# CalciferZh/MinimalOptiX

Hardware: AMD Instinct MI355X
Metric: Mrays/s (primary+bounce+shadow rays traced per second, coffee.obj 1920x1080 256spp) (higher is better)
Workload: dtype f32

## Files before the change

minimaloptix_amd/csrc/api_context.h:

```cpp
#pragma once
#include <hip/hip_runtime.h>

#include <initializer_list>
#include <string>
#include <vector>

#include "../../include/moptix.h"
#include "lbvh.h"
#include "megakernel.h"
#include "refitkernel.h"
#include "pt_signtopo.h"

struct ncclComm;

namespace pt { namespace api {

template <class T> struct DevBuf {
  T* p = nullptr; size_t n = 0;
  hipError_t ensure(size_t count) {
    if (count <= n && p) return hipSuccess;
    if (p) { (void)hipFree(p); p = nullptr; n = 0; }
    hipError_t e = hipMalloc((void**)&p, sizeof(T) * (count ? count : 1));
    if (e == hipSuccess) n = count ? count : 1;
    return e;
// ... 250 lines not shown
void fill_view(moptix_context c, SceneView& v);
int scene_features(moptix_context c);
int fill_query_view(moptix_context c, SceneView& v);
moptix_aov_buffers aov_ptrs(moptix_context c);
void comm_release(moptix_context c);
int denoise_begin(moptix_context c, bool ownGuide, size_t& px);
void denoise_consts(moptix_context c, const moptix_denoise_params* p, DenoiseConsts& k);
inline float* denoise_out(moptix_context c) { return c->dn.bound ? c->dn.bound : c->dn.out.p; }

struct LaunchPlan {
  const TraceKernel* kernel;
  int variant;
  int features;
  int nItems, tilesX;
  int nBlocks;
  long long perPass;
  int slotsInUse, auxDepth, drainBelow, ovfDepth;
  int tileMajor, unitShift; long long historyUnits;
  size_t poolBytes, overflowInts, workInts;
};
struct RenderLaunch {
  LaunchPlan p; LaunchArgs a;
  long long perPass;
  bool counted, fast;
};
struct PassOverride {
  const int* order; int nWork;
  hipError_t (*reduce)(hipStream_t stream, const LaunchArgs& a, void* user); void* user;
};
int prepare_launch(moptix_context c, int32_t nSeeds, bool counted, bool byPixelSlots, RenderLaunch& r);
int launch_pass(moptix_context c, RenderLaunch& r, const int* dSeeds, int n, const PassOverride* over);

}}
```

minimaloptix_amd/csrc/api_render.hip:

```cpp
#include <rocprim/rocprim.hpp>

#include <algorithm>
#include <cstdio>
#include <cstdlib>
#include <cstring>

#include "api_context.h"
#include "pt_lanestack.h"

using namespace pt;
using namespace pt::api;

namespace {

constexpr int kProbeWidth = 128;
int choose_node_format(moptix_context c) {
  c->formatDecided = true;
  c->nodeFormatUsed = 128;
  for (auto& v : c->probeCounts) v = 0;
  if (c->bvh.nNodes <= 0 || !c->bvh.nodes64) return MOPTIX_OK;
  if (c->opt.nodeFormat != 0) { c->nodeFormatUsed = c->opt.nodeFormat; return MOPTIX_OK; }
  SceneView v; fill_view(c, v);
  v.nodes64 = c->bvh.nodes64;
  const int w = std::min(kProbeWidth, v.width), h = std::max(1, (int)((long long)v.height * w / std::max(1, v.width)));
// ... 85 lines not shown
  const long long localTiles = (nTiles + c->nRanks - 1) / c->nRanks;
  if (localTiles * 64 > 0x7fffffffLL) return fail(c, MOPTIX_ERR_LIMIT, "frame too large");
  p.nItems = (int)(localTiles * 64); p.tilesX = tilesX;
  if (p.nItems == 0) return MOPTIX_OK;
  const long long budget = (long long)c->opt.sampleBufMB << 20;
  p.perPass = budget / ((long long)p.nItems * 12);
  p.nBlocks = c->numCUs * c->opt.blocksPerCU;
  const long long counterSlack = (long long)c->numCUs * std::max(4, c->opt.blocksPerCU) * 1024 + 65536;
  if ((long long)p.nItems + counterSlack > 0x7fffffffLL) return fail(c, MOPTIX_ERR_LIMIT, "frame too large");
  p.perPass = std::min(p.perPass, (0x7fffffffLL - counterSlack) / p.nItems);
  p.perPass = std::max(1LL, std::min(p.perPass, (long long)nSeeds));

  const bool hasTris = scene.rootRef != kEmptyRef;
  const bool analyticQueue = c->opt.analyticQueue >= 0 ? c->opt.analyticQueue != 0 : (c->spheres.size() + c->quads.size() >= 64);
  const bool packetOk = hasTris && scene.nLights <= 3 && !scene.anyDisneyAnalytic;
  const double nSamples = (double)p.nItems * (double)nSeeds;
  const bool autoPacket = nSamples >= 1.0e6 && nSeeds >= 16;
  const bool variantExplicit = c->opt.kernelVariant >= 0;
  const int variant = variantExplicit ? c->opt.kernelVariant : 3;
  const bool usePacket = packetOk && (variant == 4 || (!variantExplicit && c->opt.autoPacket != 0 && autoPacket));
  const bool useQueue = !usePacket && (byPixelSlots || ((variant >= 3) && (hasTris || analyticQueue)));
  p.kernel = usePacket ? &kPacketKernel : !useQueue ? nullptr : hasTris ? &kQueueKernel : &kLeanQueueKernel;
  p.variant = usePacket ? 4 : useQueue ? 3 : 0;
  p.features = (usePacket && c->opt.specialize != 0) ? scene_features(c) : FEAT_ALL;
  if (p.kernel == &kLeanQueueKernel && c->opt.blocksPerCU == 3) p.nBlocks = c->numCUs * 4;
  p.slotsInUse = c->opt.slotsInUse >= 0 ? c->opt.slotsInUse : (usePacket && c->opt.auxDepth > 0 && nSamples < 1.0e8 && c->glassFaceShare <= 0.5 ? packetkernel_slots() * 7 / 8 : 0);
  p.auxDepth = usePacket ? c->opt.auxDepth : 0;
  if (usePacket) {
    bool glassMaterial = false;
    for (const DevMaterial& m : c->mats) if (m.kind == MAT_DISNEY && m.brdfType == BRDF_GLASS) glassMaterial = true;
    p.drainBelow = (glassMaterial && !scene.shadowNearest) ? 0 : c->opt.drainBelow;
  }
  if (p.kernel) {
    p.ovfDepth = hasTris ? std::max(0, c->bvh.stackBound - p.kernel->lds_stack_entries() + 1) : 0;
    p.overflowInts = p.ovfDepth > 0 ? p.kernel->overflow_ints(p.nBlocks, p.ovfDepth) : 0;
    p.poolBytes = p.kernel->cold_bytes(p.nBlocks);
  } else {
    p.overflowInts = lane_stack_overflow_entries((size_t)p.nBlocks * 256, c->bvh.stackBound, megakernel_lds_stack_entries());
  }
  p.workInts = 2 + drain_list_ints(p.nBlocks, p.drainBelow);
  p.tileMajor = byPixelSlots ? 3 : p.kernel ? c->opt.tileMajor : 0;
  p.unitShift = p.tileMajor == 3 ? 0 : 6;
  p.historyUnits = (localTiles * 64) >> p.unitShift;
  return MOPTIX_OK;
}

int report_tile_history(moptix_context c) {
  std::vector<unsigned int> cost((size_t)c->tiles.units);
  HIPCHK(c, hipMemcpy(cost.data(), c->tiles.keys.p, sizeof(unsigned int) * cost.size(), hipMemcpyDeviceToHost), "read tile cost");
  size_t hist[6] = { 0, 0, 0, 0, 0, 0 };
  for (size_t i = 0; i < cost.size(); i++) {
    const unsigned int v = cost[i];
    hist[v == 0 ? 0 : v < 16 ? 1 : v < 64 ? 2 : v < 256 ? 3 : 4]++;
    if (v >= 256 && i < cost.size() / 2) hist[5]++;
  }
  fprintf(stderr, "[moptix] depth history (%zu units): none %zu, depth 8-15 %zu, 16-63 %zu, 64-255 %zu, capped %zu (of which %zu in the first half)\n",
          cost.size(), hist[0], hist[1], hist[2], hist[3], hist[4], hist[5]);
  return MOPTIX_OK;
}

#ifdef PT_EVLOG
constexpr size_t kEvLogWords = 65536;
int evlog_begin(moptix_context c, DevBuf<unsigned long long>& evLog, LaunchArgs& a) {
// ... 33 lines not shown
  a.starveLanes = c->opt.starveLanes; a.swapLanes = c->opt.swapLanes;
  a.slotsInUse = p.slotsInUse; a.auxDepth = p.auxDepth; a.ovfDepth = p.ovfDepth;
  a.watchdogTicks = (unsigned long long)c->opt.watchdogMs * 100000ull;
  if (p.overflowInts > 0) {
    HIPCHK(c, c->dOverflow.ensure(p.overflowInts), "alloc stack overflow area");
    a.stackOverflow = c->dOverflow.p;
  }
  if (p.kernel) {
    HIPCHK(c, c->dPoolCold.ensure(p.poolBytes), "alloc path pool");
    a.poolCold = c->dPoolCold.p;
  }
  long long perPass = p.perPass;
  for (;;) {
    const hipError_t e = c->dSampleBuf.ensure((size_t)perPass * a.nItems * 3);
    if (e == hipSuccess) break;
    if (e != hipErrorOutOfMemory || perPass <= 1) return hipFail(c, e, "alloc per-sample buffer");
    (void)hipGetLastError();
    perPass = (perPass + 1) / 2;
  }
  r.perPass = perPass;
  a.sampleBuf = c->dSampleBuf.p;
  HIPCHK(c, c->dWork.ensure(p.workInts), "alloc work counter");
  {
    const int hdr[2 + kDrainEntries] = { 0, 0, 0, 0, 0, 0, p.nBlocks * p.drainBelow, p.drainBelow };
    HIPCHK(c, hipMemcpyAsync(c->dWork.p, hdr, sizeof(hdr), hipMemcpyHostToDevice, c->stream), "init work counter");
    HIPCHK(c, hipStreamSynchronize(c->stream), "sync");
  }
  a.workCounter = c->dWork.p;
  a.tileMajor = p.tileMajor; a.unitShift = p.unitShift;
  if (p.tileMajor) {
    HIPCHK(c, c->tiles.ensure(p.historyUnits, c->stream), "start depth history");
    a.tileOrder = c->tiles.order.p; a.tileCost = c->tiles.keys.p;
  }
  if (counted) {
    HIPCHK(c, c->dCounters.ensure(kCntTotal), "alloc counters");
    HIPCHK(c, hipMemsetAsync(c->dCounters.p, 0, sizeof(unsigned long long) * kCntTotal, c->stream), "zero counters");
    HIPCHK(c, hipMemsetAsync(c->dCounters.p + kCntFirstWaveIn, 0xff, sizeof(unsigned long long) * 2, c->stream), "init min counters");
    a.counters = c->dCounters.p;
  }
  return MOPTIX_OK;
}

static hipError_t sort_pairs_desc(void* tmp, size_t& tmpBytes, OrderList& l, size_t n, hipStream_t stream) {
  return rocprim::radix_sort_pairs_desc(tmp, tmpBytes, l.keys.p, l.keysSorted.p, l.iota.p, l.order.p, n, 0, 32, stream);
}

hipError_t OrderList::ensure(long long n, hipStream_t stream) {
  if (units == n) return hipSuccess;
  units = -1;
  std::vector<int> ids((size_t)n);
  for (size_t i = 0; i < ids.size(); i++) ids[i] = (int)i;
  hipError_t e = keys.ensure((size_t)n);
  if (e == hipSuccess) e = keysSorted.ensure((size_t)n);
  if (e == hipSuccess) e = order.ensure((size_t)n);
  if (e == hipSuccess) e = iota.upload(ids, stream);
  if (e == hipSuccess) e = hipMemsetAsync(keys.p, 0, sizeof(unsigned int) * (size_t)n, stream);
  size_t tmpBytes = 0;
  if (e == hipSuccess) e = sort_pairs_desc(nullptr, tmpBytes, *this, (size_t)n, stream);
  if (e == hipSuccess) e = sortTmp.ensure(tmpBytes);
  if (e == hipSuccess) e = hipStreamSynchronize(stream);
  if (e == hipSuccess) units = n;
  return e;
}

hipError_t OrderList::sort(hipStream_t stream) {
  size_t tmpBytes = sortTmp.n;
  return sort_pairs_desc(sortTmp.p, tmpBytes, *this, (size_t)units, stream);
}

int launch_pass(moptix_context c, RenderLaunch& r, const int* dSeeds, int n, const PassOverride* over) {
  LaunchArgs& a = r.a;
  const LaunchPlan& p = r.p;
  a.seeds = dSeeds; a.nSeeds = n; a.nWork = over ? over->nWork : n * a.nItems;
  HIPCHK(c, hipMemsetAsync(c->dWork.p, 0, (2 + kDrainCap) * sizeof(int), c->stream), "zero work counter");
  if (over) a.tileOrder = over->order;
  else if (a.tileMajor && a.tileCost) HIPCHK(c, c->tiles.sort(c->stream), "sort tiles");
  HIPCHK(c, hipEventRecord(c->ev0, c->stream), "event");
  if (p.kernel) HIPCHK(c, p.kernel->launch(c->stream, a, p.nBlocks, r.counted, r.fast, p.features), p.kernel->launchWhat);
  else HIPCHK(c, launch_megakernel(c->stream, a, p.nBlocks, r.counted), "launch megakernel");
  if (p.drainBelow > 0) HIPCHK(c, launch_drainkernel(c->stream, a, c->numCUs, r.counted, r.fast), "launch drain kernel");
  else if (p.kernel == &kPacketKernel) HIPCHK(c, launch_megakernel(c->stream, a, p.nBlocks, r.counted), "launch megakernel");
  HIPCHK(c, hipEventRecord(c->ev1, c->stream), "event");
  if (over) HIPCHK(c, over->reduce(c->stream, a, over->user), "launch adaptive reduction");
  else HIPCHK(c, launch_reduce_samples(c->stream, a), "launch sample reduction");
  HIPCHK(c, hipEventRecord(c->ev2, c->stream), "event");
  c->asyncPending = true;
  return MOPTIX_OK;
}

}}

namespace {

int do_render(moptix_context c, const int32_t* seeds, int32_t nSeeds, bool counted, bool blocking, moptix_stats* stats) {
  int rc = check_ready(c);
  if (rc != MOPTIX_OK) return rc;
  if (nSeeds < 0 || (nSeeds > 0 && !seeds)) return fail(c, MOPTIX_ERR_INVALID, "bad seeds");
// ... 26 lines not shown
}

}

extern "C" {

int moptix_launch(moptix_context c, int32_t randSeed) { return do_render(c, &randSeed, 1, false, true, nullptr); }
int moptix_render(moptix_context c, const int32_t* seeds, int32_t nSeeds) { return do_render(c, seeds, nSeeds, false, true, nullptr); }
int moptix_render_async(moptix_context c, const int32_t* seeds, int32_t nSeeds) { return do_render(c, seeds, nSeeds, false, false, nullptr); }
int moptix_render_counted(moptix_context c, const int32_t* seeds, int32_t nSeeds, moptix_stats* out) {
  if (out) memset(out, 0, sizeof(*out));
  return do_render(c, seeds, nSeeds, true, true, out);
}

int moptix_sync(moptix_context c) {
  if (!c) return MOPTIX_ERR_INVALID;
  HIPCHK(c, hipStreamSynchronize(c->stream), "stream synchronize");
  if (c->asyncPending) {
    float ms = 0.f, ms2 = 0.f;
    if (hipEventElapsedTime(&ms, c->ev0, c->ev1) == hipSuccess) { c->kernelMs += ms; c->nLaunches++; }
    if (hipEventElapsedTime(&ms2, c->ev1, c->ev2) == hipSuccess) c->reduceMs += ms2;
    c->asyncPending = false;
    int flags[2] = { 0, 0 };
    if (c->dWork.p) HIPCHK(c, hipMemcpy(flags, c->dWork.p, sizeof(flags), hipMemcpyDeviceToHost), "read watchdog flag");
    if (flags[1] != 0) return fail(c, MOPTIX_ERR_HIP, "render kernel hit its watchdog (option watchdog_ms); this pass was not added to accuBuffer");
  }
  return MOPTIX_OK;
}

}
```

minimaloptix_amd/csrc/lbvh.hip:

```cpp
#include <cstring>
#include <utility>
#include <vector>
#include <hip/hip_runtime.h>
#include <rocprim/rocprim.hpp>

#include "lbvh.h"
#include "pt_lbvh.h"

namespace pt {

namespace {

constexpr int kBlock = 256;
inline int grid_for(int n) { return (n + kBlock - 1) / kBlock; }

struct SceneBox { uint32_t cLo[3], cHi[3], sLo[3], sHi[3]; };

constexpr int kReplicas = 64;
__global__ void k_init_box(SceneBox* b) {
  b += blockIdx.x;
  if (threadIdx.x < 3) {
    b->cLo[threadIdx.x] = float_to_ordered(1e37f); b->cHi[threadIdx.x] = float_to_ordered(-1e37f);
    b->sLo[threadIdx.x] = float_to_ordered(1e37f); b->sHi[threadIdx.x] = float_to_ordered(-1e37f);
  }
// ... 52 lines not shown
  const v3 shi = mk3(ordered_to_float(box->sHi[0]), ordered_to_float(box->sHi[1]), ordered_to_float(box->sHi[2]));
  keys[f] = morton_key(c, clo, invExt, lbvh_bits_per_axis(n), lbvh_index_bits(n), f) | (tri_is_big(l, h, slo, shi) ? 0ull : kSmallKeyBit);
}

__global__ void k_leaves(int n, const uint64_t* __restrict__ keys, const float* __restrict__ facePos,
                         const float* __restrict__ faceNrm, const int* __restrict__ faceHasNrm, const int* __restrict__ faceMat,
                         const float* __restrict__ lo, const float* __restrict__ hi, const SceneBox* box,
                         Tri48* __restrict__ tris, TriShade* __restrict__ shade, float* __restrict__ leafLo, float* __restrict__ leafHi) {
  const int k = blockIdx.x * blockDim.x + threadIdx.x;
  if (k >= n) return;
  const int f = key_face(keys[k], lbvh_index_bits(n));
  const float* p = facePos + 9 * (size_t)f;
  const v3 p0 = mk3(p[0], p[1], p[2]), p1 = mk3(p[3], p[4], p[5]), p2 = mk3(p[6], p[7], p[8]);
  Tri48 t;
  t.p0 = p0; t.e0 = p1 - p0; t.e1 = p0 - p2; t.mat = faceMat[f] & ((1 << kFaceMatBits) - 1); t.prim = f; t.shadow = faceMat[f] >> kFaceMatBits;
  tris[k] = t;
  TriShade sh;
  sh.n0 = mk3(0, 0, 0); sh.n1 = sh.n0; sh.n2 = sh.n0; sh.hasNormals = 0; sh.pad1 = 0; sh.pad2 = 0;
  if (faceNrm != nullptr && faceHasNrm != nullptr && faceHasNrm[f]) {
    const float* q = faceNrm + 9 * (size_t)f;
    sh.n0 = mk3(q[0], q[1], q[2]); sh.n1 = mk3(q[3], q[4], q[5]); sh.n2 = mk3(q[6], q[7], q[8]); sh.hasNormals = 1;
  }
  shade[k] = sh;
  const float ex = ordered_to_float(box->sHi[0]) - ordered_to_float(box->sLo[0]);
  const float ey = ordered_to_float(box->sHi[1]) - ordered_to_float(box->sLo[1]);
  const float ez = ordered_to_float(box->sHi[2]) - ordered_to_float(box->sLo[2]);
  const float padAbs = 1e-5f * fmaxf_(fmaxf_(ex, ey), ez) + 1e-30f;
  for (int a = 0; a < 3; a++) { leafLo[3 * k + a] = pad_lo(lo[3 * f + a], padAbs); leafHi[3 * k + a] = pad_hi(hi[3 * f + a], padAbs); }
}

__global__ void k_karras(int n, const uint64_t* __restrict__ keys, int* __restrict__ left, int* __restrict__ right,
                         int* __restrict__ first, int* __restrict__ last, int* __restrict__ parentI, int* __restrict__ parentL) {
  const int i = blockIdx.x * blockDim.x + threadIdx.x;
  if (i >= n - 1) return;
  const KarrasNode kn = karras_node(keys, n, i);
  left[i] = kn.left; right[i] = kn.right; first[i] = kn.first; last[i] = kn.last;
  if (kn.left < 0) parentL[~kn.left] = i; else parentI[kn.left] = i;
  if (kn.right < 0) parentL[~kn.right] = i; else parentI[kn.right] = i;
  if (i == 0) parentI[0] = -1;
}

struct SahTask { int node, first, count; float cbLo[3], cbHi[3]; int force; };
constexpr int kWideTasks = 1024;
constexpr int kWideCount = 2048;
constexpr int kCbReplicas = 32;

// ... 370 lines not shown

  float *lo = nullptr, *hi = nullptr, *leafLo = nullptr, *leafHi = nullptr, *ilo = nullptr, *ihi = nullptr;
  uint64_t *keys = nullptr, *keysSorted = nullptr;
  int *left = nullptr, *right = nullptr, *first = nullptr, *last = nullptr, *parentI = nullptr, *parentL = nullptr, *kept = nullptr, *newIndex = nullptr, *opened = nullptr;
  unsigned int* arrivals = nullptr; SceneBox* box = nullptr; int* dDepth = nullptr; void* tmp = nullptr;
  int *order = nullptr, *orderTmp = nullptr, *sahFlags = nullptr, *sahOffs = nullptr, *sahNext = nullptr, *sahLeft = nullptr, *sahLeftScan = nullptr;
  SahBins* sahBins = nullptr; SahSplit* sahSplits = nullptr; uint32_t* sahChildCb = nullptr;
  SahTask *tasksA = nullptr, *tasksB = nullptr, *sahChildren = nullptr;
  size_t tmpSah = 0;
  size_t tmpSort = 0, tmpScan = 0, tmpBytes = 0;
  hipEvent_t e0 = nullptr, e1 = nullptr;
  std::vector<std::pair<int, int> > levelRange;
  int* pinned = nullptr;

  LB_CHECK(hipEventCreate(&e0)); LB_CHECK(hipEventCreate(&e1));
  LB_CHECK(hipHostMalloc((void**)&pinned, 8 * sizeof(int), hipHostMallocDefault));
  LB_CHECK(dmalloc(&lo, 3 * (size_t)n)); LB_CHECK(dmalloc(&hi, 3 * (size_t)n));
  LB_CHECK(dmalloc(&leafLo, 3 * (size_t)n)); LB_CHECK(dmalloc(&leafHi, 3 * (size_t)n));
  LB_CHECK(dmalloc(&ilo, 3 * (size_t)ni)); LB_CHECK(dmalloc(&ihi, 3 * (size_t)ni));
  LB_CHECK(dmalloc(&keys, (size_t)n)); LB_CHECK(dmalloc(&keysSorted, (size_t)n));
  LB_CHECK(dmalloc(&left, (size_t)ni)); LB_CHECK(dmalloc(&right, (size_t)ni)); LB_CHECK(dmalloc(&first, (size_t)ni)); LB_CHECK(dmalloc(&last, (size_t)ni));
  LB_CHECK(dmalloc(&parentI, (size_t)ni)); LB_CHECK(dmalloc(&parentL, (size_t)n)); LB_CHECK(dmalloc(&kept, (size_t)ni + 1)); LB_CHECK(dmalloc(&newIndex, (size_t)ni + 1)); LB_CHECK(dmalloc(&opened, 2 * (size_t)ni + 2));
  LB_CHECK(dmalloc(&arrivals, (size_t)ni)); LB_CHECK(dmalloc(&box, (size_t)kReplicas)); LB_CHECK(dmalloc(&dDepth, 1));
  LB_CHECK(dmalloc(&out->tris, (size_t)n)); LB_CHECK(dmalloc(&out->shade, (size_t)n));
  LB_CHECK(rocprim::radix_sort_keys(nullptr, tmpSort, keys, keysSorted, (size_t)n, 0, 64, stream));
  if (ni > 0) LB_CHECK(rocprim::exclusive_scan(nullptr, tmpScan, kept, newIndex, 0, (size_t)ni, rocprim::plus<int>(), stream));
  if (builder == 1 && n > leafSize) {
    LB_CHECK(dmalloc(&order, (size_t)n)); LB_CHECK(dmalloc(&orderTmp, (size_t)n));
    LB_CHECK(dmalloc(&sahFlags, (size_t)n + 2)); LB_CHECK(dmalloc(&sahOffs, (size_t)n + 2)); LB_CHECK(dmalloc(&sahNext, 2));
    LB_CHECK(dmalloc(&sahLeft, (size_t)n + 1)); LB_CHECK(dmalloc(&sahLeftScan, (size_t)n + 1));
    LB_CHECK(dmalloc(&sahBins, (size_t)kWideTasks)); LB_CHECK(dmalloc(&sahSplits, (size_t)kWideTasks)); LB_CHECK(dmalloc(&sahChildCb, 12 * (size_t)kWideTasks * kCbReplicas));
    LB_CHECK(dmalloc(&tasksA, (size_t)n / 2 + 2)); LB_CHECK(dmalloc(&tasksB, (size_t)n / 2 + 2)); LB_CHECK(dmalloc(&sahChildren, (size_t)n + 2));
    LB_CHECK(rocprim::exclusive_scan(nullptr, tmpSah, sahFlags, sahOffs, 0, (size_t)n + 2, rocprim::plus<int>(), stream));
    if (tmpSah > tmpScan) tmpScan = tmpSah;
  }
  tmpBytes = tmpSort > tmpScan ? tmpSort : tmpScan;
  LB_CHECK(hipMalloc(&tmp, tmpBytes ? tmpBytes : 16));

  LB_CHECK(hipEventRecord(e0, stream));
  k_init_box<<<kReplicas, 64, 0, stream>>>(box);
  k_bounds<<<grid_for(n), kBlock, 0, stream>>>(n, dFacePos, lo, hi, box);
  k_fold_box<<<1, 64, 0, stream>>>(box);
  k_morton<<<grid_for(n), kBlock, 0, stream>>>(n, lo, hi, box, keys);
  LB_CHECK(rocprim::radix_sort_keys(tmp, tmpSort, keys, keysSorted, (size_t)n, 0, 64, stream));
  if (builder == 1 && n > leafSize) {
    k_sah_init<<<grid_for(n), kBlock, 0, stream>>>(n, keysSorted, order, tasksA, box);
    LB_CHECK(hipMemsetAsync(parentI, 0xff, sizeof(int) * (size_t)ni, stream));
// ... 87 lines not shown
```

minimaloptix_amd/csrc/megakernel.h:

```cpp
#pragma once
#include <hip/hip_runtime.h>
#include "pt_counters.h"
#include "pt_types.h"

namespace pt {

struct LaunchArgs {
  SceneView scene;
  const int* seeds; int nSeeds;
  float* accum;
  float* sampleBuf;
  int* workCounter;
  int nItems;
  int nWork;
  int tilesX; int rank, nRanks;
  int exitThreshold;
  int leafThreshold;
  int* stackOverflow;
  unsigned long long* counters;
  void* poolCold;
  int starveLanes;
  int swapLanes;
  int ovfDepth;
  int slotsInUse;
  int auxDepth;
  unsigned long long watchdogTicks;
  int tileMajor;
  int unitShift;
  const int* tileOrder;
  unsigned int* tileCost;
#ifdef PT_EVLOG
  unsigned long long* evLog;
#endif
};
constexpr int kDeepPath = 8;
constexpr int kDrainDeep = 24;
constexpr int kDrainList = 2, kDrainDeepN = 0, kDrainNext = 1, kDrainOtherN = 2, kDrainCap = 4, kDrainBelow = 5, kDrainEntries = 6;

#if defined(__HIPCC__)
__device__ __forceinline__ bool item_to_pixel(const LaunchArgs& a, int k, int& sample, int& pixel) {
  sample = k / a.nItems;
  const int i = k - sample * a.nItems;
  const int lt = i >> 6, in = i & 63;
  const int gt = lt * a.nRanks + (a.rank + lt) % a.nRanks;
  const int tx = gt % a.tilesX, ty = gt / a.tilesX;
  const int x = tx * 8 + (in & 7), y = ty * 8 + (in >> 3);
  pixel = y * a.scene.width + x;
  return (x < a.scene.width) & (y < a.scene.height);
}
__device__ __forceinline__ int handout_to_item(const LaunchArgs& a, int k) {
  if (!a.tileMajor) return k;
  if (a.tileMajor == 3) {
    const int ui = k / a.nSeeds, sample = k - ui * a.nSeeds;
    return sample * a.nItems + (a.tileOrder ? a.tileOrder[ui] : ui);
  }
  const int per = a.nSeeds << 6;
  const int ti = k / per, r = k - ti * per;
  const int lt = a.tileOrder ? a.tileOrder[ti] : ti;
  if (a.tileMajor == 2) {
    const int in = r / a.nSeeds, sample = r - in * a.nSeeds;
    return sample * a.nItems + (lt << 6) + in;
  }
  return (r >> 6) * a.nItems + (lt << 6) + (r & 63);
}
__device__ __forceinline__ void store_sample(const LaunchArgs& a, int item, v3 value) {
  float* sp = a.sampleBuf + 3 * (size_t)item;
  sp[0] = value.x; sp[1] = value.y; sp[2] = value.z;
}
#endif

int megakernel_lds_stack_entries();
hipError_t launch_reduce_samples(hipStream_t stream, const LaunchArgs& a);
hipError_t launch_megakernel(hipStream_t stream, const LaunchArgs& a, int nBlocks, bool counted);
int queuekernel_lds_stack_entries();
int queuekernel_slots();
size_t queuekernel_cold_bytes(int nBlocks);
size_t queuekernel_overflow_ints(int nBlocks, int ovfDepth);
hipError_t launch_queuekernel(hipStream_t stream, const LaunchArgs& a, int nBlocks, bool counted, bool fastShading, int features);
int queuekernel_lds_stack_entries_lean();
int queuekernel_slots_lean();
size_t queuekernel_cold_bytes_lean(int nBlocks);
size_t queuekernel_overflow_ints_lean(int nBlocks, int ovfDepth);
hipError_t launch_queuekernel_lean(hipStream_t stream, const LaunchArgs& a, int nBlocks, bool counted, bool fastShading, int features);
int packetkernel_lds_stack_entries();
int packetkernel_slots();
size_t packetkernel_cold_bytes(int nBlocks);
size_t packetkernel_overflow_ints(int nBlocks, int ovfDepth);
// ... 20 lines not shown
```

minimaloptix_amd/csrc/packetkernel_body.h:

```cpp
  constexpr int NS = SHARED ? kP * kWaves : kP;
  __shared__ PoolLds<NS> sPool[SHARED ? 1 : kWaves];
  __shared__ WavePriv<NS> sPriv[kWaves];
#ifdef PT_EVLOG
  __shared__ int sEvOn;
  if (threadIdx.x == 0) sEvOn = 0;
#define PT_EV(code, val) do { if (sEvOn && (threadIdx.x & 63) == 0) { const unsigned long long i_ = atomicAdd(a.evLog, 1ull); \
    if (i_ < 65000ull) a.evLog[1 + i_] = (__builtin_amdgcn_s_memrealtime() << 24) | (((unsigned long long)(val) & 0xffffull) << 8) | ((unsigned long long)(threadIdx.x >> 6) << 4) | (unsigned long long)(code); } } while (0)
#else
#define PT_EV(code, val) do { } while (0)
#endif

  SceneView scv = a.scene;
  scv.shadowNearest = NEAR ? 1 : 0;
  const SceneView& sc = scv;
  const int lane = threadIdx.x & 63, wave = threadIdx.x >> 6;
  PoolLds<NS>& W = sPool[SHARED ? 0 : wave];
  const int gpool = SHARED ? blockIdx.x : blockIdx.x * kWaves + wave;
  SlotCold* cold = reinterpret_cast<SlotCold*>(a.poolCold) + (size_t)gpool * NS;
  int* ovfBase = a.stackOverflow ? a.stackOverflow + (size_t)gpool * NS * a.ovfDepth : nullptr;

  unsigned long long tLocal = 0, tLock = 0, tTxn = 0, tIdle = 0, tBLoad = 0, tBRun = 0, tBStore = 0, nTxn = 0, nIter = 0;
  unsigned long long tSub = 0, nIterResult = 0, nIterLights = 0, nIterGen = 0, nodeRuns = 0, ringBacklog = 0, leafBacklog = 0;
#define PT_SUB0() do { if (CNT) tSub = __builtin_amdgcn_s_memtime(); } while (0)
#define PT_SUB(acc) do { if (CNT) { const unsigned long long now_ = __builtin_amdgcn_s_memtime(); acc += now_ - tSub; tSub = now_; } } while (0)
// ... 297 lines not shown
    __builtin_amdgcn_s_waitcnt(0); PT_EV(2, 0);
#endif
    for (;;) {
      if (have && ps.mode == M_NEW_SAMPLE) {
        if (CNT) {
          const unsigned long long b = min((unsigned long long)(kCntTailBuckets - 1), (__builtin_amdgcn_s_memrealtime() - rtStart) / 100000ull);
          atomicAdd(a.counters + kCntTailCount + b, 1ull); atomicMax(a.counters + kCntTailMaxDepth + b, (unsigned long long)ps.depth); atomicAdd(a.counters + kCntTailDepthSum + b, (unsigned long long)ps.depth);
        }
        store_sample(a, ps.item, ps.accum);
        if (CNT) atomicAdd(a.counters + kCntPacketFinished, 1ull);
        if (a.tileCost != nullptr && ps.depth >= kDeepPath) atomicMax(a.tileCost + ((ps.item % a.nItems) >> a.unitShift), (unsigned int)ps.depth);
        ps.mode = M_NEW_PIXEL;
      }
      const bool resultFirst = __ballot(have && ps.mode == M_RESULT) != 0ull;
      const bool run = have && ps.mode != M_TRACE && ps.mode != M_DONE &&
                       !((shadeBatch || resultFirst) && ps.mode == M_NEW_PIXEL);
      if (__ballot(run) == 0ull) break;
      if (CNT) {
        if (__ballot(run && ps.mode == M_RESULT)) nIterResult++;
        if (__ballot(run && ps.mode == M_NEW_PIXEL)) nIterGen++;
      }
      if (run) {
        if (ps.mode == M_RESULT) {
          on_result_packet<CNT, FAST, SlotSink, F>(sc, ps, pk, res, att, ct, sink);
        } else {
          int k = atomicAdd(a.workCounter, 1);
          k = (k >= a.nWork) ? -1 : handout_to_item(a, k);
          if (CNT && k < 0) atomicMin(a.counters + kCntItemsRanOut, (unsigned long long)__builtin_amdgcn_s_memrealtime());
          int s;
          if (k < 0) { ps.mode = M_DONE; }
          else if (item_to_pixel(a, k, s, ps.pixel)) { ps.item = k; begin_sample<CNT>(sc, ps, a.seeds[s], ct); packet_primary(pk); }
        }
      }
    }
    if (CNT) { __builtin_amdgcn_s_waitcnt(0); PT_SUB(tBRun); }
#ifdef PT_EVLOG
    __builtin_amdgcn_s_waitcnt(0); PT_EV(3, 0);
#endif
    bool useAux = false;
    if (have) {
      SlotCold* cw = at32(cold, slot);
      if (axp >= 0 && !(ps.mode == M_TRACE && ps.depth >= a.auxDepth)) {
        for (int j = 0; j < kPacketShadows; j++) { const int ax = (axp >> (kSlotBits * j)) & kSlotMask; atomicOr(&W.freeMask[ax >> 5], 1u << (ax & 31)); }
        atomicAdd(&W.nFree, kPacketShadows);
        axp = -1;
      }
      int axpNext = axp;
      if (auxOn) {
        const bool wantAux = axp < 0 && ps.mode == M_TRACE && ps.depth >= a.auxDepth;
        if (wantAux && W.nFree >= kPacketShadows) {
          int got = 0, pack = 0;
          for (int wi = 0; wi < NS / 32 && got < kPacketShadows; wi++) {
            unsigned int cur = W.freeMask[wi];
            while (cur != 0u && got < kPacketShadows) {
// ... 256 lines not shown
```

minimaloptix_amd/csrc/pt_path.h:

```cpp
#pragma once
#include "pt_types.h"
#include "pt_rng.h"
#include "pt_geom.h"
#include "pt_disney.h"
#include "pt_texture.h"

namespace pt {

enum { M_NEW_PIXEL = 0, M_NEW_SAMPLE = 1, M_TRACE = 2, M_RESULT = 3, M_LIGHTS = 4, M_DONE = 5 };
enum { RK_RADIANCE = 0, RK_SHADOW = 1 };

struct Counters {
  uint32_t samples, primaryRays, bounceRays, shadowRays;
  uint32_t nodeFetches, triTests, closestHits, lightLoads, analyticTests;
  uint32_t censusLanes[kCensusRegions], censusWaves[kCensusRegions];
};
template <bool CNT> PT_HD void cnt(uint32_t& c, uint32_t n = 1) { if (CNT) c += n; }
enum { CR_RESULT = 0, CR_MISS, CR_HIT, CR_LIGHT, CR_DEPTHCAP, CR_LAMBERT, CR_METAL, CR_GLASS, CR_DISNEY_GLASS, CR_DISNEY, CR_LIGHT0, CR_LIGHT1,
       CR_LIGHT2, CR_BOUNCE_EVAL, CR_GEN, CR_TRI0, CR_TRI1, CR_TRI2, CR_TRI3, CR_TRI_HIT, CR_SHADOW_FOLD, CR_LIGHT_DRAW, CR_BOUNCE_SAMPLE, CR_NODE_BRANCHED };
template <bool CNT> PT_HD void census(Counters& ct, int region) {
#if defined(__HIP_DEVICE_COMPILE__)
  if constexpr (CNT) {
    const unsigned long long m = __ballot(1);
    ct.censusLanes[region]++;
// ... 325 lines not shown
          }
        }
      }
    }
    if (terminated) tv.node = kTravDone;
    else trav_pop(tv, st);
  }
}
template <bool CNT, class Stack>
PT_HD void trav_leaf_step(const SceneView& sc, const PathState& ps, Trav& tv, Stack& st, Counters& ct) {
  LeafChunk ch;
  leaf_fetch4(sc, tv.node, 0, ch);
  trav_leaf_step_fetched<CNT>(sc, ps, tv, st, ct, ch);
}

template <bool CNT, bool N64 = false, class Stack>
PT_HD void trav_step(const SceneView& sc, const PathState& ps, Trav& tv, Stack& st, Counters& ct) {
  if (tv.node >= 0) trav_node_step<CNT, N64>(sc, ps, tv, st, ct);
  else trav_leaf_step<CNT>(sc, ps, tv, st, ct);
}


template <bool CNT>
PT_HD void begin_sample(const SceneView& sc, PathState& ps, int launchSeed, Counters& ct) {
  const int x = ps.pixel % sc.width, y = ps.pixel / sc.width;
  ps.depth = 1;
  ps.seed = tea16((uint32_t)y * (uint32_t)sc.width + (uint32_t)x, (uint32_t)launchSeed);
  ps.thr = mk3(1.f, 1.f, 1.f); ps.rad = mk3(0.f, 0.f, 0.f);
  const v3 randInLens = rand_in_unit_disk(ps.seed) * sc.cam.lensRadius;
  const v3 offs = sc.cam.u * randInLens.x + sc.cam.v * randInLens.y;
  const float r1 = rnd(ps.seed); const float r2 = rnd(ps.seed);
  const float xyx = ((float)x + r1 - 0.5f) / (float)sc.width;
  const float xyy = ((float)y + r2 - 0.5f) / (float)sc.height;
  ps.o = sc.cam.origin + offs;
  ps.d = normalize((((sc.cam.scrLowerLeftCorner + sc.cam.horizontal * xyx) + sc.cam.vertical * xyy) - sc.cam.origin) - offs);
  ps.tmin = sc.epsT; ps.tmax = kRtDefaultMax; ps.kind = RK_RADIANCE;
  ps.mode = M_TRACE;
  cnt<CNT>(ct.samples); cnt<CNT>(ct.primaryRays); census<CNT>(ct, CR_GEN);
}

PT_HD void end_sample(PathState& ps) {
  ps.accum = mk3(clampf(ps.rad.x, 0.f, 1.f), clampf(ps.rad.y, 0.f, 1.f), clampf(ps.rad.z, 0.f, 1.f));
  ps.mode = M_NEW_SAMPLE;
}

PT_HD void bounce(const SceneView& sc, PathState& ps, v3 o, v3 d, uint32_t childSeed) {
  ps.o = o; ps.d = d; ps.tmin = sc.epsT; ps.tmax = kRtDefaultMax; ps.kind = RK_RADIANCE;
  ps.depth++; ps.seed = childSeed;
  ps.mode = M_TRACE;
}

template <bool CNT>
PT_HD void glass_body(const SceneView& sc, PathState& ps, float ior, v3 tint, const HitAttr& h, Counters& ct) {
  v3 normal = h.shadingNormal;
  float cosThetaI = -dot(ps.d, normal);
  float refIdx;
  if (cosThetaI > 0.f) { refIdx = ior; }
  else { refIdx = 1.f / ior; cosThetaI = -cosThetaI; normal = -normal; }
  v3 refracted;
  const bool totalReflection = !refract(refracted, ps.d, normal, refIdx);
  const float cosThetaT = -dot(normal, refracted);
  const float reflectProb = totalReflection ? 1.f : fresnel(cosThetaI, cosThetaT, refIdx);
  const uint32_t childSeed = fork_seed(ps.seed, ps.depth + 1);
  v3 no, nd;
  if (rnd(ps.seed) < reflectProb) { no = h.front; nd = reflect(ps.d, normal); }
  else { no = h.back; nd = refracted; }
  ps.thr = ps.thr * tint;
  cnt<CNT>(ct.bounceRays);
  bounce(sc, ps, no, nd, childSeed);
}

template <int F = FEAT_ALL>
PT_HD void hit_attributes(const SceneView& sc, const PathState& ps, const Trav& tv, HitAttr& h) {
  const float t = tv.tbest;
  if (has<F>(FEAT_SPHERES) && tv.bestPrim < sc.nSpheres) {
    const DevSphere s = sc.spheres[tv.bestPrim];
    const v3 p = ray_at(ps.o, ps.d, t);
    h.geoNormal = normalize(p - s.center);
    h.shadingNormal = h.geoNormal;
    h.texu = 0.f; h.texv = 0.f;
    h.front = p; h.back = p;
    h.mat = sc.sphereMat[tv.bestPrim];
  } else if (tv.bestPrim < sc.nSpheres + sc.nQuads) {
    const DevQuad* q = sc.quads + (tv.bestPrim - sc.nSpheres);
    const v3 n = xyz(q->plane);
    h.geoNormal = n; h.shadingNormal = n;
    h.texu = 0.f; h.texv = 0.f;
    h.front = ray_at(ps.o, ps.d, t); h.back = h.front;
    h.mat = q->mat;
  } else {
    const Tri48 tpv = load_const(at32(sc.tris, tv.bestTri));
    const TriShade spv = load_const(at32(sc.triShade, tv.bestTri));
    const Tri48* tp = &tpv;
    const TriShade* sp = &spv;
    const v3 p0 = tp->p0, e0 = tp->e0, e1 = tp->e1;
    const v3 sn0 = sp->n0, sn1 = sp->n1, sn2 = sp->n2;
    const int hasNormals = sp->hasNormals;
// ... 157 lines not shown
```

minimaloptix_amd/csrc/pt_types.h:

```cpp
#pragma once
#include "pt_math.h"

namespace pt {

constexpr int kMaxLeaf = 8;
template <class T>
PT_HD T load_const(const T* p) {
#if defined(__HIP_DEVICE_COMPILE__)
  static_assert(sizeof(T) % 4 == 0, "whole dwords");
  typedef __attribute__((address_space(4))) const unsigned int cu32;
  cu32* w = (cu32*)reinterpret_cast<const unsigned int*>(p);
  T out;
  unsigned int* o = reinterpret_cast<unsigned int*>(&out);
#pragma unroll
  for (unsigned i = 0; i < sizeof(T) / 4; i++) o[i] = w[i];
  return out;
#else
  return *p;
#endif
}
template <class T> PT_HD T load_uniform(const T* p) { return load_const(p); }
template <class T> PT_HD T* at32(T* table, int index) {
#if defined(__HIP_DEVICE_COMPILE__)
  return reinterpret_cast<T*>(reinterpret_cast<char*>(table) + (uint32_t)((uint32_t)index * (uint32_t)sizeof(T)));
// ... 29 lines not shown

struct alignas(64) Node64 {
  float ox, oy, oz;
  float sx, sy, sz;
  uint32_t q[6];
  int ref[4];
};
static_assert(sizeof(Node64) == 64, "Node64 must be 64 bytes");

struct alignas(16) Tri48 {
  v3 p0; int mat;
  v3 e0; int prim;
  v3 e1; int shadow;
};
static_assert(sizeof(Tri48) == 48, "Tri48 must be 48 bytes");

struct alignas(16) TriShade {
  v3 n0; int hasNormals;
  v3 n1; int pad1;
  v3 n2; int pad2;
};
static_assert(sizeof(TriShade) == 48, "TriShade must be 48 bytes");

struct alignas(16) TriUV { float u0, v0, u1, v1, u2, v2; int hasUV; int pad; };
static_assert(sizeof(TriUV) == 32, "TriUV must be 32 bytes");

struct DevTexture { const v4* texels; int width, height; };

struct alignas(16) DevQuad {
  v4 plane;
  v3 v1; int mat;
  v3 v2; int pad0;
  v3 anchor; int pad1;
};
static_assert(sizeof(DevQuad) == 64, "DevQuad must be 64 bytes");

struct alignas(16) DevSphere { v3 center; float radius; };
static_assert(sizeof(DevSphere) == 16, "DevSphere must be 16 bytes");

struct alignas(16) DevLight {
  v3 position; float area;
  v3 normal;   float radius;
  v3 emission; int shape;
  v3 u; int pad0;
  v3 v; int pad1;
};
static_assert(sizeof(DevLight) == 80, "DevLight must be 80 bytes");

enum { MAT_LAMBERTIAN = 0, MAT_METAL = 1, MAT_GLASS = 2, MAT_DISNEY = 3, MAT_LIGHT = 4 };
enum { BRDF_NORMAL = 0, BRDF_GLASS = 1 };
enum { LIGHT_SPHERE = 0, LIGHT_QUAD = 1 };
enum { FEAT_TEXTURE = 1, FEAT_SPHERE_LIGHT = 2, FEAT_PLAIN_MATERIALS = 4, FEAT_SPHERES = 8, FEAT_ALL = 15 };
template <int F> PT_HD constexpr bool has(int bit) { return (F & bit) != 0; }
enum { SHADOW_NONE = 0, SHADOW_OPAQUE = 1, SHADOW_GLASS = 2 };
PT_HD int shadow_class(int kind, int brdfType) { return kind != MAT_DISNEY ? SHADOW_NONE : (brdfType == BRDF_GLASS ? SHADOW_GLASS : SHADOW_OPAQUE); }
constexpr int kFaceMatBits = 28;
PT_HD int face_mat_word(int mat, int shadow) { return mat | (shadow << kFaceMatBits); }

struct alignas(16) DevMaterial {
  int kind; int brdfType; float fuzz; float refIdx;
  v3 albedo;   float metallic;
  v3 emission; float roughness;
  v3 color;    float subsurface;
  v3 Cdlin;    float sheen;
  v3 Cspec0;   float clearcoat;
  v3 Csheen;   float oneMinusMetallic;
  float diffuseRatio;
  float specAlpha;
  float ccAlpha;
  float ccRatio;
  float ax, ay;
  float ccA2m1;
  float ccPiLogA2;
  int albedoTex;
  float specular, specularTint, sheenTint;
};
static_assert(sizeof(DevMaterial) == 160, "DevMaterial layout");

struct Cam { v3 origin, horizontal, vertical, scrLowerLeftCorner, u, v; float lensRadius; };

struct SceneView {
  int width, height;
  int maxDepth; float minIntensity; float epsT;
  v3 bg;
  Cam cam;
  int nSpheres; const DevSphere* spheres; const int* sphereMat;
  int nQuads;   const DevQuad* quads;
  int nLights;  const DevLight* lights;
  int nMaterials; const DevMaterial* mats;
  int anyDisneyAnalytic;
  int shadowNearest;
  int nTris; int rootRef;
  const Node128* nodes; const Tri48* tris; const TriShade* triShade;
  const Node64* nodes64;
  const TriUV* triUV;
  int nTextures; const DevTexture* textures;
};

}
```

minimaloptix_amd/csrc/refitkernel.hip:

```cpp
#include <hip/hip_runtime.h>

#include "refitkernel.h"

namespace pt {

namespace {

constexpr int kBlock = 256;
constexpr int kLevelBlock = 64;
inline int grid_for(int n, int block) { return (n + block - 1) / block; }

__global__ void k_refit_box_init(uint32_t* box) {
  if (threadIdx.x < kRefitBoxWords) box[blockIdx.x * kRefitBoxWords + threadIdx.x] = float_to_ordered(threadIdx.x < 3 ? 1e37f : -1e37f);
}
__global__ void k_refit_box_fold(uint32_t* box) {
  const int w = threadIdx.x;
  if (w >= kRefitBoxWords) return;
  uint32_t v = box[w];
  for (int r = 1; r < kRefitBoxReplicas; r++) { const uint32_t x = box[r * kRefitBoxWords + w]; v = w < 3 ? min(v, x) : max(v, x); }
  box[w] = v;
}

__device__ __forceinline__ float wave_min(float v) {
#pragma unroll
  for (int o = 32; o >= 1; o >>= 1) v = fminf_(v, __shfl_xor(v, o));
  return v;
}
__device__ __forceinline__ float wave_max(float v) {
#pragma unroll
  for (int o = 32; o >= 1; o >>= 1) v = fmaxf_(v, __shfl_xor(v, o));
  return v;
}

__global__ void __launch_bounds__(kBlock) k_refit_tris(const RefitArgs a) {
  const int k = blockIdx.x * kBlock + threadIdx.x;
  float l[3] = { 1e37f, 1e37f, 1e37f }, h[3] = { -1e37f, -1e37f, -1e37f };
  if (k < a.nTris) {
    Tri48 old;
    old.mat = a.tris[k].mat; old.prim = a.tris[k].prim; old.shadow = a.tris[k].shadow;
    const int f = old.prim;
    const bool hasNrm = a.faceNrm != nullptr && a.faceHasNrm != nullptr && a.faceHasNrm[f] != 0;
    Tri48 t; TriShade sh; RefitBox raw;
    refit_triangle(a.facePos + 9 * (size_t)f, a.faceNrm + 9 * (size_t)f, hasNrm, old, t, sh, raw);
    a.tris[k] = t; a.shade[k] = sh; a.raw[k] = raw;
    l[0] = raw.lox; l[1] = raw.loy; l[2] = raw.loz; h[0] = raw.hix; h[1] = raw.hiy; h[2] = raw.hiz;
  }
  const float v[6] = { wave_min(l[0]), wave_min(l[1]), wave_min(l[2]), wave_max(h[0]), wave_max(h[1]), wave_max(h[2]) };
  if ((threadIdx.x & 63) == 0) {
    uint32_t* box = a.sceneBox + (blockIdx.x % kRefitBoxReplicas) * kRefitBoxWords;
    for (int i = 0; i < 3; i++) { atomicMin(&box[i], float_to_ordered(v[i])); atomicMax(&box[3 + i], float_to_ordered(v[3 + i])); }
  }
}

__device__ __forceinline__ float scene_pad_abs(const uint32_t* box) {
  return refit_pad_abs(mk3(ordered_to_float(box[0]), ordered_to_float(box[1]), ordered_to_float(box[2])),
                       mk3(ordered_to_float(box[3]), ordered_to_float(box[4]), ordered_to_float(box[5])));
}

__global__ void __launch_bounds__(kLevelBlock) k_refit_level(const RefitArgs a, int first, int count) {
  const int i = blockIdx.x * kLevelBlock + threadIdx.x;
  if (i >= count) return;
  const int n = a.levelOrder[first + i];
  const float padAbs = scene_pad_abs(a.sceneBox);
  Node128 nd = a.nodes[n];
  refit_node(nd, a.raw, padAbs, a.nodes);
  a.nodes[n] = nd;
  if (a.nodes64 != nullptr) {
// ... 71 lines not shown
```

Baseline: 9027.

## Add packed per-triangle face records and magic-division work handout for specialized packet kernel

Builds a 64-byte TriFace record per triangle, holding first vertex, vertex normals, geometric normal and material, appended after the TriShade array and written at BVH build and refit. When the packet kernel is specialized with no optional features, hit attributes for triangles are read from this single aligned record, avoiding separate Tri48/TriShade fetches and the cross-product normalization. It also precomputes magic-number divisors stored ahead of the work counter, so the work handout avoids integer divisions. This costs extra memory and extra writes per triangle at build and refit, and adds another host sync when the pass seed count changes.

```diff
diff --git a/minimaloptix_amd/csrc/api_context.h b/minimaloptix_amd/csrc/api_context.h
--- a/minimaloptix_amd/csrc/api_context.h
+++ b/minimaloptix_amd/csrc/api_context.h
@@ -296,6 +296,7 @@
 struct RenderLaunch {
   LaunchPlan p; LaunchArgs a;
   long long perPass;
+  int handoutDivisor, handoutSeeds;
   bool counted, fast;
 };
 struct PassOverride {
diff --git a/minimaloptix_amd/csrc/api_render.hip b/minimaloptix_amd/csrc/api_render.hip
--- a/minimaloptix_amd/csrc/api_render.hip
+++ b/minimaloptix_amd/csrc/api_render.hip
@@ -131,7 +131,8 @@
   const bool useQueue = !usePacket && (byPixelSlots || ((variant >= 3) && (hasTris || analyticQueue)));
   p.kernel = usePacket ? &kPacketKernel : !useQueue ? nullptr : hasTris ? &kQueueKernel : &kLeanQueueKernel;
   p.variant = usePacket ? 4 : useQueue ? 3 : 0;
-  p.features = (usePacket && c->opt.specialize != 0) ? scene_features(c) : FEAT_ALL;
+  const bool faceTableOk = (unsigned long long)tri_face_offset(0) + (unsigned long long)scene.nTris * (sizeof(TriShade) + sizeof(TriFace)) + 64ull < (1ull << 32);
+  p.features = (usePacket && c->opt.specialize != 0 && faceTableOk) ? scene_features(c) : FEAT_ALL;
   if (p.kernel == &kLeanQueueKernel && c->opt.blocksPerCU == 3) p.nBlocks = c->numCUs * 4;
   p.slotsInUse = c->opt.slotsInUse >= 0 ? c->opt.slotsInUse : (usePacket && c->opt.auxDepth > 0 && nSamples < 1.0e8 && c->glassFaceShare <= 0.5 ? packetkernel_slots() * 7 / 8 : 0);
   p.auxDepth = usePacket ? c->opt.auxDepth : 0;
@@ -147,7 +148,7 @@
   } else {
     p.overflowInts = lane_stack_overflow_entries((size_t)p.nBlocks * 256, c->bvh.stackBound, megakernel_lds_stack_entries());
   }
-  p.workInts = 2 + drain_list_ints(p.nBlocks, p.drainBelow);
+  p.workInts = kHandoutWords + 2 + drain_list_ints(p.nBlocks, p.drainBelow);
   p.tileMajor = byPixelSlots ? 3 : p.kernel ? c->opt.tileMajor : 0;
   p.unitShift = p.tileMajor == 3 ? 0 : 6;
   p.historyUnits = (localTiles * 64) >> p.unitShift;
@@ -227,11 +228,14 @@
   a.sampleBuf = c->dSampleBuf.p;
   HIPCHK(c, c->dWork.ensure(p.workInts), "alloc work counter");
   {
-    const int hdr[2 + kDrainEntries] = { 0, 0, 0, 0, 0, 0, p.nBlocks * p.drainBelow, p.drainBelow };
-    HIPCHK(c, hipMemcpyAsync(c->dWork.p, hdr, sizeof(hdr), hipMemcpyHostToDevice, c->stream), "init work counter");
+    struct { HandoutConsts hc; int hdr[2 + kDrainEntries]; } w = { handout_consts(p.tileMajor, a.nItems, (int)std::min<long long>(perPass, nSeeds), a.tilesX, a.nRanks),
+                                                                   { 0, 0, 0, 0, 0, 0, p.nBlocks * p.drainBelow, p.drainBelow } };
+    static_assert(sizeof(w) == sizeof(int) * (kHandoutWords + 2 + kDrainEntries), "the work header is packed");
+    HIPCHK(c, hipMemcpyAsync(c->dWork.p, &w, sizeof(w), hipMemcpyHostToDevice, c->stream), "init work counter");
     HIPCHK(c, hipStreamSynchronize(c->stream), "sync");
-  }
-  a.workCounter = c->dWork.p;
+    r.handoutDivisor = handout_divisor(p.tileMajor, a.nItems, (int)std::min<long long>(perPass, nSeeds)); r.handoutSeeds = (int)std::min<long long>(perPass, nSeeds);
+  }
+  a.workCounter = c->dWork.p + kHandoutWords;
   a.tileMajor = p.tileMajor; a.unitShift = p.unitShift;
   if (p.tileMajor) {
     HIPCHK(c, c->tiles.ensure(p.historyUnits, c->stream), "start depth history");
@@ -277,7 +281,13 @@
   LaunchArgs& a = r.a;
   const LaunchPlan& p = r.p;
   a.seeds = dSeeds; a.nSeeds = n; a.nWork = over ? over->nWork : n * a.nItems;
-  HIPCHK(c, hipMemsetAsync(c->dWork.p, 0, (2 + kDrainCap) * sizeof(int), c->stream), "zero work counter");
+  if (handout_divisor(a.tileMajor, a.nItems, n) != r.handoutDivisor || n != r.handoutSeeds) {
+    const HandoutConsts hc = handout_consts(a.tileMajor, a.nItems, n, a.tilesX, a.nRanks);
+    HIPCHK(c, hipMemcpyAsync(a.workCounter - kHandoutWords, &hc, sizeof(hc), hipMemcpyHostToDevice, c->stream), "write hand-out constants");
+    HIPCHK(c, hipStreamSynchronize(c->stream), "sync");
+    r.handoutDivisor = handout_divisor(a.tileMajor, a.nItems, n); r.handoutSeeds = n;
+  }
+  HIPCHK(c, hipMemsetAsync(a.workCounter, 0, (2 + kDrainCap) * sizeof(int), c->stream), "zero work counter");
   if (over) a.tileOrder = over->order;
   else if (a.tileMajor && a.tileCost) HIPCHK(c, c->tiles.sort(c->stream), "sort tiles");
   HIPCHK(c, hipEventRecord(c->ev0, c->stream), "event");
@@ -350,7 +360,7 @@
     if (hipEventElapsedTime(&ms2, c->ev1, c->ev2) == hipSuccess) c->reduceMs += ms2;
     c->asyncPending = false;
     int flags[2] = { 0, 0 };
-    if (c->dWork.p) HIPCHK(c, hipMemcpy(flags, c->dWork.p, sizeof(flags), hipMemcpyDeviceToHost), "read watchdog flag");
+    if (c->dWork.p) HIPCHK(c, hipMemcpy(flags, c->dWork.p + kHandoutWords, sizeof(flags), hipMemcpyDeviceToHost), "read watchdog flag");
     if (flags[1] != 0) return fail(c, MOPTIX_ERR_HIP, "render kernel hit its watchdog (option watchdog_ms); this pass was not added to accuBuffer");
   }
   return MOPTIX_OK;
diff --git a/minimaloptix_amd/csrc/lbvh.hip b/minimaloptix_amd/csrc/lbvh.hip
--- a/minimaloptix_amd/csrc/lbvh.hip
+++ b/minimaloptix_amd/csrc/lbvh.hip
@@ -98,6 +98,7 @@
     sh.n0 = mk3(q[0], q[1], q[2]); sh.n1 = mk3(q[3], q[4], q[5]); sh.n2 = mk3(q[6], q[7], q[8]); sh.hasNormals = 1;
   }
   shade[k] = sh;
+  *tri_face_slot(shade, n, k) = make_tri_face(t, sh);
   const float ex = ordered_to_float(box->sHi[0]) - ordered_to_float(box->sLo[0]);
   const float ey = ordered_to_float(box->sHi[1]) - ordered_to_float(box->sLo[1]);
   const float ez = ordered_to_float(box->sHi[2]) - ordered_to_float(box->sLo[2]);
@@ -514,7 +515,8 @@
   LB_CHECK(dmalloc(&left, (size_t)ni)); LB_CHECK(dmalloc(&right, (size_t)ni)); LB_CHECK(dmalloc(&first, (size_t)ni)); LB_CHECK(dmalloc(&last, (size_t)ni));
   LB_CHECK(dmalloc(&parentI, (size_t)ni)); LB_CHECK(dmalloc(&parentL, (size_t)n)); LB_CHECK(dmalloc(&kept, (size_t)ni + 1)); LB_CHECK(dmalloc(&newIndex, (size_t)ni + 1)); LB_CHECK(dmalloc(&opened, 2 * (size_t)ni + 2));
   LB_CHECK(dmalloc(&arrivals, (size_t)ni)); LB_CHECK(dmalloc(&box, (size_t)kReplicas)); LB_CHECK(dmalloc(&dDepth, 1));
-  LB_CHECK(dmalloc(&out->tris, (size_t)n)); LB_CHECK(dmalloc(&out->shade, (size_t)n));
+  LB_CHECK(dmalloc(&out->tris, (size_t)n));
+  LB_CHECK(hipMalloc((void**)&out->shade, (size_t)tri_face_offset(n) + sizeof(TriFace) * (size_t)n));
   LB_CHECK(rocprim::radix_sort_keys(nullptr, tmpSort, keys, keysSorted, (size_t)n, 0, 64, stream));
   if (ni > 0) LB_CHECK(rocprim::exclusive_scan(nullptr, tmpScan, kept, newIndex, 0, (size_t)ni, rocprim::plus<int>(), stream));
   if (builder == 1 && n > leafSize) {
diff --git a/minimaloptix_amd/csrc/megakernel.h b/minimaloptix_amd/csrc/megakernel.h
--- a/minimaloptix_amd/csrc/megakernel.h
+++ b/minimaloptix_amd/csrc/megakernel.h
@@ -37,8 +37,7 @@
 constexpr int kDrainDeep = 24;
 constexpr int kDrainList = 2, kDrainDeepN = 0, kDrainNext = 1, kDrainOtherN = 2, kDrainCap = 4, kDrainBelow = 5, kDrainEntries = 6;
 
-#if defined(__HIPCC__)
-__device__ __forceinline__ bool item_to_pixel(const LaunchArgs& a, int k, int& sample, int& pixel) {
+PT_HD bool item_to_pixel(const LaunchArgs& a, int k, int& sample, int& pixel) {
   sample = k / a.nItems;
   const int i = k - sample * a.nItems;
   const int lt = i >> 6, in = i & 63;
@@ -48,7 +47,7 @@
   pixel = y * a.scene.width + x;
   return (x < a.scene.width) & (y < a.scene.height);
 }
-__device__ __forceinline__ int handout_to_item(const LaunchArgs& a, int k) {
+PT_HD int handout_to_item(const LaunchArgs& a, int k) {
   if (!a.tileMajor) return k;
   if (a.tileMajor == 3) {
     const int ui = k / a.nSeeds, sample = k - ui * a.nSeeds;
@@ -63,6 +62,52 @@
   }
   return (r >> 6) * a.nItems + (lt << 6) + (r & 63);
 }
+struct MagicDiv { unsigned int mul, shift; };
+struct HandoutConsts { MagicDiv first, tilesX, ranks, seeds; };
+constexpr int kHandoutWords = 8;
+static_assert(sizeof(HandoutConsts) == kHandoutWords * sizeof(int), "HandoutConsts is kHandoutWords ints");
+inline MagicDiv magic_div(int d) {
+  int l = 0;
+  while ((1ll << l) < (long long)d) l++;
+  MagicDiv m; m.shift = 31u + (unsigned int)l;
+  m.mul = (unsigned int)(((1ull << m.shift) + (unsigned long long)d - 1ull) / (unsigned long long)d);
+  return m;
+}
+PT_HD int magic_quot(int n, MagicDiv m) { return (int)(((unsigned long long)(unsigned int)n * (unsigned long long)m.mul) >> m.shift); }
+inline int handout_divisor(int tileMajor, int nItems, int nSeeds) { return !tileMajor ? nItems : tileMajor == 3 ? nSeeds : nSeeds << 6; }
+inline HandoutConsts handout_consts(int tileMajor, int nItems, int nSeeds, int tilesX, int nRanks) {
+  HandoutConsts h;
+  h.first = magic_div(handout_divisor(tileMajor, nItems, nSeeds)); h.tilesX = magic_div(tilesX); h.ranks = magic_div(nRanks); h.seeds = magic_div(nSeeds);
+  return h;
+}
+
+struct WorkItem { int item, sample, x, y, pixel; };
+PT_HD bool handout_lean(const LaunchArgs& a, const HandoutConsts* hc, int k, WorkItem& w) {
+  int slot;
+  const int q = magic_quot(k, load_uniform(&hc->first));
+  if (!a.tileMajor) {
+    w.sample = q; slot = k - q * a.nItems;
+  } else if (a.tileMajor == 3) {
+    w.sample = k - q * a.nSeeds;
+    slot = a.tileOrder ? a.tileOrder[q] : q;
+  } else {
+    const int r = k - q * (a.nSeeds << 6);
+    const int lt = a.tileOrder ? a.tileOrder[q] : q;
+    int in;
+    if (a.tileMajor == 2) { in = magic_quot(r, load_uniform(&hc->seeds)); w.sample = r - in * a.nSeeds; }
+    else { w.sample = r >> 6; in = r & 63; }
+    slot = (lt << 6) + in;
+  }
+  w.item = a.tileMajor ? w.sample * a.nItems + slot : k;
+  const int lt = slot >> 6, in = slot & 63;
+  int gt = lt;
+  if (__builtin_expect(a.nRanks != 1, 0)) { const int s = a.rank + lt; gt = lt * a.nRanks + (s - magic_quot(s, load_uniform(&hc->ranks)) * a.nRanks); }
+  const int ty = magic_quot(gt, load_uniform(&hc->tilesX)), tx = gt - ty * a.tilesX;
+  w.x = tx * 8 + (in & 7); w.y = ty * 8 + (in >> 3);
+  w.pixel = w.y * a.scene.width + w.x;
+  return (w.x < a.scene.width) & (w.y < a.scene.height);
+}
+#if defined(__HIPCC__)
 __device__ __forceinline__ void store_sample(const LaunchArgs& a, int item, v3 value) {
   float* sp = a.sampleBuf + 3 * (size_t)item;
   sp[0] = value.x; sp[1] = value.y; sp[2] = value.z;
diff --git a/minimaloptix_amd/csrc/packetkernel_body.h b/minimaloptix_amd/csrc/packetkernel_body.h
--- a/minimaloptix_amd/csrc/packetkernel_body.h
+++ b/minimaloptix_amd/csrc/packetkernel_body.h
@@ -343,14 +343,21 @@
       }
       if (run) {
         if (ps.mode == M_RESULT) {
-          on_result_packet<CNT, FAST, SlotSink, F>(sc, ps, pk, res, att, ct, sink);
+          on_result_packet<CNT, FAST, SlotSink, (F == 0 && !N64) ? FEAT_SPLIT_HIT : F>(sc, ps, pk, res, att, ct, sink);
         } else {
           int k = atomicAdd(a.workCounter, 1);
+          if constexpr (F == 0) {
+            const HandoutConsts* hc = reinterpret_cast<const HandoutConsts*>(a.workCounter) - 1;
+            WorkItem w;
+            if (k >= a.nWork) { ps.mode = M_DONE; }
+            else if (handout_lean(a, hc, k, w)) { ps.pixel = w.pixel; ps.item = w.item; begin_sample_xy<CNT>(sc, ps, w.x, w.y, a.seeds[w.sample], ct); packet_primary(pk); }
+          } else {
           k = (k >= a.nWork) ? -1 : handout_to_item(a, k);
           if (CNT && k < 0) atomicMin(a.counters + kCntItemsRanOut, (unsigned long long)__builtin_amdgcn_s_memrealtime());
           int s;
           if (k < 0) { ps.mode = M_DONE; }
           else if (item_to_pixel(a, k, s, ps.pixel)) { ps.item = k; begin_sample<CNT>(sc, ps, a.seeds[s], ct); packet_primary(pk); }
+          }
         }
       }
     }
diff --git a/minimaloptix_amd/csrc/pt_path.h b/minimaloptix_amd/csrc/pt_path.h
--- a/minimaloptix_amd/csrc/pt_path.h
+++ b/minimaloptix_amd/csrc/pt_path.h
@@ -371,8 +371,7 @@
 
 
 template <bool CNT>
-PT_HD void begin_sample(const SceneView& sc, PathState& ps, int launchSeed, Counters& ct) {
-  const int x = ps.pixel % sc.width, y = ps.pixel / sc.width;
+PT_HD void begin_sample_xy(const SceneView& sc, PathState& ps, int x, int y, int launchSeed, Counters& ct) {
   ps.depth = 1;
   ps.seed = tea16((uint32_t)y * (uint32_t)sc.width + (uint32_t)x, (uint32_t)launchSeed);
   ps.thr = mk3(1.f, 1.f, 1.f); ps.rad = mk3(0.f, 0.f, 0.f);
@@ -386,6 +385,11 @@
   ps.tmin = sc.epsT; ps.tmax = kRtDefaultMax; ps.kind = RK_RADIANCE;
   ps.mode = M_TRACE;
   cnt<CNT>(ct.samples); cnt<CNT>(ct.primaryRays); census<CNT>(ct, CR_GEN);
+}
+template <bool CNT>
+PT_HD void begin_sample(const SceneView& sc, PathState& ps, int launchSeed, Counters& ct) {
+  const int x = ps.pixel % sc.width, y = ps.pixel / sc.width;
+  begin_sample_xy<CNT>(sc, ps, x, y, launchSeed, ct);
 }
 
 PT_HD void end_sample(PathState& ps) {
@@ -419,9 +423,24 @@
   bounce(sc, ps, no, nd, childSeed);
 }
 
+PT_HD void hit_attributes_face(const SceneView& sc, const PathState& ps, const Trav& tv, HitAttr& h) {
+  const TriFace fv = load_const(tri_face(sc, tv.bestTri));
+  h.mat = fv.matNrm & 0x7fffffff;
+  h.texu = 0.f; h.texv = 0.f;
+  h.geoNormal = fv.gn;
+  if (fv.matNrm < 0) {
+    const v3 n0 = mk3(fv.n0x, fv.n0y, fv.n0z), n1 = mk3(fv.n1x, fv.n1y, fv.n1z), n2 = mk3(fv.n2x, fv.n2y, fv.n2z);
+    h.shadingNormal = normalize((n1 * tv.beta + n2 * tv.gamma) + n0 * (1.f - tv.beta - tv.gamma));
+  } else {
+    h.shadingNormal = h.geoNormal;
+  }
+  refine_hitpoint(ray_at(ps.o, ps.d, tv.tbest), ps.d, h.geoNormal, fv.p0, h.back, h.front);
+}
+
 template <int F = FEAT_ALL>
 PT_HD void hit_attributes(const SceneView& sc, const PathState& ps, const Trav& tv, HitAttr& h) {
   const float t = tv.tbest;
+  if constexpr (F == 0) { if (tv.bestPrim >= sc.nSpheres + sc.nQuads) { hit_attributes_face(sc, ps, tv, h); return; } }
   if (has<F>(FEAT_SPHERES) && tv.bestPrim < sc.nSpheres) {
     const DevSphere s = sc.spheres[tv.bestPrim];
     const v3 p = ray_at(ps.o, ps.d, t);
diff --git a/minimaloptix_amd/csrc/pt_types.h b/minimaloptix_amd/csrc/pt_types.h
--- a/minimaloptix_amd/csrc/pt_types.h
+++ b/minimaloptix_amd/csrc/pt_types.h
@@ -75,6 +75,23 @@
 };
 static_assert(sizeof(TriShade) == 48, "TriShade must be 48 bytes");
 
+struct alignas(64) TriFace {
+  v3 p0; float n0x;
+  float n0y, n0z, n1x, n1y;
+  float n1z, n2x, n2y, n2z;
+  v3 gn; int matNrm;
+};
+static_assert(sizeof(TriFace) == 64, "TriFace must be 64 bytes");
+PT_HD uint32_t tri_face_offset(int nTris) { return ((uint32_t)nTris * (uint32_t)sizeof(TriShade) + 63u) & ~63u; }
+PT_HD TriFace* tri_face_slot(TriShade* shade, int nTris, int tri) { return reinterpret_cast<TriFace*>(reinterpret_cast<char*>(shade) + tri_face_offset(nTris)) + tri; }
+PT_HD TriFace make_tri_face(const Tri48& t, const TriShade& sh) {
+  TriFace f;
+  f.gn = normalize(cross(t.e1, t.e0)); f.matNrm = t.mat | (sh.hasNormals ? (int)0x80000000u : 0);
+  f.p0 = t.p0; f.n0x = sh.n0.x; f.n0y = sh.n0.y; f.n0z = sh.n0.z;
+  f.n1x = sh.n1.x; f.n1y = sh.n1.y; f.n1z = sh.n1.z; f.n2x = sh.n2.x; f.n2y = sh.n2.y; f.n2z = sh.n2.z;
+  return f;
+}
+
 struct alignas(16) TriUV { float u0, v0, u1, v1, u2, v2; int hasUV; int pad; };
 static_assert(sizeof(TriUV) == 32, "TriUV must be 32 bytes");
 
@@ -104,6 +121,7 @@
 enum { BRDF_NORMAL = 0, BRDF_GLASS = 1 };
 enum { LIGHT_SPHERE = 0, LIGHT_QUAD = 1 };
 enum { FEAT_TEXTURE = 1, FEAT_SPHERE_LIGHT = 2, FEAT_PLAIN_MATERIALS = 4, FEAT_SPHERES = 8, FEAT_ALL = 15 };
+constexpr int FEAT_SPLIT_HIT = 16;
 template <int F> PT_HD constexpr bool has(int bit) { return (F & bit) != 0; }
 enum { SHADOW_NONE = 0, SHADOW_OPAQUE = 1, SHADOW_GLASS = 2 };
 PT_HD int shadow_class(int kind, int brdfType) { return kind != MAT_DISNEY ? SHADOW_NONE : (brdfType == BRDF_GLASS ? SHADOW_GLASS : SHADOW_OPAQUE); }
@@ -149,5 +167,8 @@
   const TriUV* triUV;
   int nTextures; const DevTexture* textures;
 };
+PT_HD const TriFace* tri_face(const SceneView& sc, int tri) {
+  return reinterpret_cast<const TriFace*>(reinterpret_cast<const char*>(sc.triShade) + (uint32_t)(tri_face_offset(sc.nTris) + ((uint32_t)tri << 6)));
+}
 
 }
diff --git a/minimaloptix_amd/csrc/refitkernel.hip b/minimaloptix_amd/csrc/refitkernel.hip
--- a/minimaloptix_amd/csrc/refitkernel.hip
+++ b/minimaloptix_amd/csrc/refitkernel.hip
@@ -42,7 +42,7 @@
     const bool hasNrm = a.faceNrm != nullptr && a.faceHasNrm != nullptr && a.faceHasNrm[f] != 0;
     Tri48 t; TriShade sh; RefitBox raw;
     refit_triangle(a.facePos + 9 * (size_t)f, a.faceNrm + 9 * (size_t)f, hasNrm, old, t, sh, raw);
-    a.tris[k] = t; a.shade[k] = sh; a.raw[k] = raw;
+    a.tris[k] = t; a.shade[k] = sh; *tri_face_slot(a.shade, a.nTris, k) = make_tri_face(t, sh); a.raw[k] = raw;
     l[0] = raw.lox; l[1] = raw.loy; l[2] = raw.loz; h[0] = raw.hix; h[1] = raw.hiy; h[2] = raw.hiz;
   }
   const float v[6] = { wave_min(l[0]), wave_min(l[1]), wave_min(l[2]), wave_max(h[0]), wave_max(h[1]), wave_max(h[2]) };
```

After: 9142 (median of 6 runs). +1.3%, better.
